# thuml/HashGAN

Measured on AMD Instinct MI355X. Metric: queries/sec (mAP@R of Q queries vs N-code database, Hamming ranking), higher is better.
Workload: dtype fp4 (E2M1 0/+-1) x fp4 -> f32 exact distances; u32 xor+popcount elsewhere; f64 AP; 1 GPU; C2: Q=10000 N=1000000 b=64 R=5000 C=10, planted codes; parallelism=1 GPU

## Files before the change

hashgan_amd/csrc/hg_core.hip:

```cpp
#include "hg_ctx.hpp"
#include "hg_host_pack.hpp"
#include "hg_dev_in.hpp"
#include "hg_dev_out.hpp"

#include <exception>
#include <map>
#include <mutex>
#include <thread>
#include <unistd.h>

thread_local std::string g_err;

int fail(int code, const char* fmt, ...) {
    char buf[512];
    va_list ap;
    va_start(ap, fmt);
    vsnprintf(buf, sizeof buf, fmt, ap);
    va_end(ap);
    g_err = buf;
    return code;
}

const char* const kKernelNames[KI_COUNT] = {"k_hist", "k_hist_reduce", "k_plan", "k_seg_counts", "k_seg_layout", "k_guess",
                                            "k_select", "k_rank_hist", "k_order", "k_rank_fused", "k_match", "k_ap", "k_merge", "k_pack",
// ... 1098 lines not shown
    flag("staged_lists", &Options::staged_lists),
    flag("step_graph", &Options::step_graph),
    ranged("step_streams", &Options::step_streams, 1, 2, "step_streams must be 1 or 2"),
    ranged("timing_every", &Options::timing_every, 1, 1024, "timing_every must be 1..1024"),
    flag("host_pack", &Options::host_pack),
    ranged("keep_floats", &Options::keep_floats, 0, 2, "keep_floats must be 0, 1 or 2"),
    ranged("keep_query_floats", &Options::keep_query_floats, 0, 1, "keep_query_floats must be 0 or 1"),
    ranged("real_mfma", &Options::real_mfma, 0, 2, "real_mfma must be 0, 1 or 2"),
    flag("real_sample_half", &Options::real_sample_half),
    flag("real_second_sample", &Options::real_second_sample),
    flag("real_sort_lds", &Options::real_sort_lds),
    flag("real_groups", &Options::real_groups),
    flag("real_map_lists", &Options::real_map_lists),
    ranged("real_whole_rounds", &Options::real_whole_rounds, 0, 8, "real_whole_rounds must be 0 .. 8"),
};
}

int hg_set_option(hg_ctx* c, const char* key, int64_t value) {
    if (!c || !key) return fail(HG_ERR_ARG, "hg_set_option: null argument");
    if (!strcmp(key, "handicap_next_bet")) {
        if (value < 0 || value > 64) return fail(HG_ERR_ARG, "handicap_next_bet must be 0..64");
        c->handicap_next = value;
        return HG_OK;
    }
    if (!strcmp(key, "optimistic")) {
        c->opt.optimistic = value != 0;
        c->bet_consecutive_fail = c->shard_bet_fail = 0;
        c->cfg_epoch++;
        return HG_OK;
    }
    if (!strcmp(key, "cap_boost")) {
        if (value < 1 || value > 4096) return fail(HG_ERR_ARG, "cap_boost must be 1..4096");
        if (value > c->cap_boost && c->shard_bet_fail > 0) c->shard_bet_fail--;
        c->cap_boost = value;
        c->cfg_epoch++;
        return HG_OK;
    }
    for (const OptionKey& k : kOptionKeys) {
        if (strcmp(key, k.key)) continue;
        if (!k.flag && (value < k.lo || value > k.hi)) return fail(HG_ERR_ARG, "%s", k.range);
        c->opt.*k.field = k.flag ? value != 0 : value;
        c->cfg_epoch++;
        return HG_OK;
    }
    return fail(HG_ERR_ARG, "hg_set_option: unknown key '%s'", key);
}

int hg_trim(hg_ctx* c) {
    if (!c) return fail(HG_ERR_ARG, "hg_trim: null context");
    HG_TRY(c->use());
    HG_TRY(c->sync());
    c->for_each_buf([](DevBuf& d, BufClass k) { if (k != BUF_TABLE) d.release(); });
    c->forget_derived();
    if (c->sub) { hg_ctx* s = c->sub; c->sub = nullptr; (void)hg_destroy(s); }
    c->stage &= (ST_DB | ST_Q);
    c->lists_valid = false;
    c->real_lists = false;
    cache_release_all();
    return HG_OK;
}

int hg_preload(hg_ctx* c) {
    if (!c) return fail(HG_ERR_ARG, "hg_preload: null context");
    HG_TRY(c->use());
    HG_TRY(ensure_stream2(c));
    HG_TRY(ensure_fstage(c));
    HG_TRY(ensure_pin(c, (size_t)1 << 20));
    hipFuncAttributes a;
    HG_HIP(hipFuncGetAttributes(&a, reinterpret_cast<const void*>(&k_ap<AP_THREADS>)));
    HG_TRY(preload_seq()); HG_TRY(preload_rank()); HG_TRY(preload_side()); HG_TRY(preload_valu()); HG_TRY(preload_mx()); HG_TRY(preload_mx1()); HG_TRY(preload_real()); HG_TRY(preload_rerank());
    host_pack_warm();
    return HG_OK;
}

int hg_release_cache(void) {
    cache_release_all();
    return HG_OK;
}

int hg_get_stat(hg_ctx* c, const char* key, int64_t* value) {
    if (!c || !key || !value) return fail(HG_ERR_ARG, "hg_get_stat: null argument");
    if (!strcmp(key, "optimistic_runs")) *value = c->bet_runs;
    else if (!strcmp(key, "optimistic_fallbacks")) *value = c->bet_fallbacks;
    else if (!strcmp(key, "optimistic_requeried")) *value = c->bet_requeried;
    else if (!strcmp(key, "optimistic_rebets")) *value = c->bet_rebets;
    else if (!strcmp(key, "rank_leftovers")) *value = c->rank_leftovers;
    else if (!strcmp(key, "select_variant")) *value = c->last_select;
    else if (!strcmp(key, "rank_variant")) *value = c->last_rank;
    else if (!strcmp(key, "hist_variant")) *value = c->last_hist;
    else if (!strcmp(key, "rank_lds_recs")) *value = c->last_lds_recs;
    else if (!strcmp(key, "slice_cap")) *value = c->cap;
    else if (!strcmp(key, "rel_hist_variant")) *value = c->last_rel_hist;
    else if (!strcmp(key, "ap_at_cutoffs")) *value = c->aa.dim;
    else if (!strcmp(key, "votes_cutoffs")) *value = c->vt.dim;
    else if (!strcmp(key, "joint_hist_grades")) *value = c->jh_G;
    else if (!strcmp(key, "joint_hist_bands")) *value = c->jh_bands;
    else if (!strcmp(key, "merged_joint_grades")) *value = c->mjh_G;
    else if (!strcmp(key, "rel_hist_current")) *value = c->rh.current(c) ? 1 : 0;
    else if (!strcmp(key, "grade_hist_current")) *value = c->gh.current(c) ? 1 : 0;
    else if (!strcmp(key, "joint_hist_current")) *value = c->jh.current(c) ? 1 : 0;
    else if (!strcmp(key, "rerank_records")) *value = c->rr_records;
    else if (!strcmp(key, "rerank_chunks")) *value = c->rr_chunks;
    else if (!strcmp(key, "rerank_groups_lds")) *value = c->rr_groups_lds;
    else if (!strcmp(key, "rerank_groups_global")) *value = c->rr_groups_global;
    else if (!strcmp(key, "export_bytes")) *value = c->export_bytes;
    else if (!strcmp(key, "export_variant")) *value = c->export_variant;
// ... 105 lines not shown
```

hashgan_amd/csrc/hg_ctx.hpp:

```cpp
#pragma once
#include "hg_kernels.hpp"
#pragma GCC visibility push(default)
#include "../../include/hashgan_amd.h"
#pragma GCC visibility pop

#include <rccl/rccl.h>
#include <atomic>
#include <chrono>
#include <cmath>
#include <cstdarg>
#include <cstdio>
#include <cstdlib>
#include <cstring>
#include <string>
#include <utility>
#include <vector>

using namespace hg;

extern thread_local std::string g_err;
int fail(int code, const char* fmt, ...);

#define HG_HIP(expr)                                                                         \
    do {                                                                                     \
// ... 167 lines not shown
    i64 min_segment = 256;
    i64 max_segments = 2048;
    i64 optimistic = 1;
    i64 sample_stride = 0;
    i64 guess_sigma = 5;
    i64 cand_budget_x10 = 40;
    i64 second_bet = 1;
    i64 crowd_probe = 1;
    i64 select_mfma = 1;
    i64 select_packed = 3;
    i64 compact_records = 1;
    i64 hist_mfma = 2;
    i64 rank_lds = 2;
    i64 rank_slices = 7000;
    i64 rank_dense = 1;
    i64 rank_dense_gbm = -1;
    i64 dense_budget_mb = 16384;
    i64 all_rows_shortcut = 1;
    i64 fuse_ap = 1;
    i64 inline_leftovers = 1;
    i64 ap_wide = 1;
    i64 ap_recip = 1;
    i64 probe_select = 0;
    i64 probe_votes = 0;
    i64 stage_sync = 1;
    i64 defer_verdict = 0;
    i64 staged_lists = 1;
    i64 step_graph = 0;
    i64 step_streams = 2;
    i64 timing_every = 1;
    i64 host_pack = 1;
    i64 keep_floats = 2;
    i64 keep_query_floats = 0;
    i64 real_mfma = 2;
    i64 real_sample_half = 1;
    i64 real_second_sample = 1;
    i64 real_sort_lds = 1;
    i64 real_groups = 1;
    i64 real_map_lists = 0;
    i64 real_whole_rounds = 3;
};

enum BufClass {
    BUF_TABLE,
    BUF_DERIVED,
    BUF_WORK,
};

struct StepBufs {
    DevBuf hist, hown, posbase, t, tguess, sstar, cnt_lt, quota, tie_before, n_lt, err, sl_start, sl_tie, sl_cnt, tot, failq,
           cand, out_idx, out_dist, mbits, ap, rel, qbad, bigq, hwq;
    DevBuf outblk;
    i64 outblk_q = -1;
    template <class F> void for_each_step_buf(F&& f) {
        for (DevBuf* d : {&hist, &hown, &posbase, &t, &tguess, &sstar, &cnt_lt, &quota, &tie_before, &n_lt, &err, &sl_start, &sl_tie,
                          &sl_cnt, &tot, &failq, &cand, &out_idx, &out_dist, &mbits, &ap, &rel, &qbad, &bigq, &hwq})
            f(*d, BUF_WORK);
        f(outblk, BUF_DERIVED);
    }
};

struct StepState {
    unsigned stage = ST_NONE;
    Geo geo{};
    i64 RW = 0;
    bool optimistic = false;
    bool lists_valid = false;
    bool rec8 = false;
    u32 cap = 0;
    i64 crow = 0;
    bool ap_fused = false;
    bool leftovers_inline = false;
    int last_select = SEL_NONE;
    int last_rank = RK_NONE;
    int last_hist = 0;
    i64 last_lds_recs = 0;
};

struct StepReq {
    bool fuse_ap = false;
    enum Rows { RECORDS, BYTES, DIRECT } rows = RECORDS;
    bool exact_cut = false;
    bool err_zeroed = false;
    i64 guess_sigma = 0;
    i64 cand_budget_x10 = 0;
    void* dst = nullptr;
};

struct RowSource;
struct RealReq {
    RowSource* src = nullptr;
    i64 R = 0;
    bool bet = false;
    double sigma = 0.0, budget = 0.0;
    bool with_ap = false;
    bool no_cut = false;
    double expect = 0.0;
    bool samp16 = false;
    bool skip_lists = false;
};

struct RealState {
    bool filtered = false;
    bool lds_ranked = false;
    bool grouped = false;
    bool lists_made = false;
    bool half = false;
    i64 attempts = 0;
// ... 295 lines not shown
inline void SideResult::finish(const hg_ctx* c, i64 Q_, i64 Qpad_, i64 dim_) { *this = SideResult{true, c->q_gen, c->db_gen, Q_, Qpad_, dim_}; }
inline bool SideResult::current(const hg_ctx* c) const { return done && q_gen == c->q_gen && db_gen == c->db_gen; }

struct FirstReservations {
    const unsigned long long e0 = g_alloc_epoch.load();
    void keep(hg_ctx* c) const { if (c->map_warm_epoch == e0) c->map_warm_epoch = g_alloc_epoch; }
};

inline int download_planes(hg_ctx* c, const DevBuf& src, size_t plane, void* const* host, int k) {
    for (int i = 0; i < k; ++i)
        if (host[i]) HG_HIP(hipMemcpyAsync(host[i], src.as<char>() + i * plane, plane, hipMemcpyDeviceToHost, c->stream));
    return HG_OK;
}
inline int download_pitched(hg_ctx* c, void* host, const DevBuf& src, i64 Q, i64 Qpad, i64 rows) {
    HG_HIP(hipMemcpy2DAsync(host, (size_t)Q * 4, src.p, (size_t)Qpad * 4, (size_t)Q * 4, (size_t)rows, hipMemcpyDeviceToHost, c->stream));
    return HG_OK;
}
inline void widen_u32(int64_t* dst, const void* src, size_t n) {
    for (size_t i = 0; i < n; ++i) dst[i] = ((const u32*)src)[i];
}

inline int grid_for(i64 n, int per_block = 256) { return (int)((n + per_block - 1) / per_block); }
inline int padded_grid(int nBlk) { return (nBlk + 7) / 8 * 8; }

int need(hg_ctx* c, unsigned st, const char* who, const char* what);
int upload_codes(hg_ctx* c, DevBuf& dst, const uint64_t* host, i64 n, int W, int NW);
int ensure_pin(hg_ctx* c, size_t need_b);
int do_match(hg_ctx* c);
int ensure_ap_tables(hg_ctx* c, bool* use_recip);
int do_ap_range(hg_ctx* c, i64 q0, i64 nq, const u32* only = nullptr);
inline int do_ap(hg_ctx* c) { return do_ap_range(c, 0, c->geo.Q); }
int ensure_out_block(hg_ctx* c);
int read_plan_flag(hg_ctx* c, int* flag);
int launch_min_topr(hg_ctx* c, const u32* idx_all, const u8* dist_all, i64 n, int G);
hg_ctx* requery_child(hg_ctx* c, i64 nF);
int stage_ap_download(hg_ctx* c, void* dst = nullptr);
int wait_verdict(hg_ctx* c, bool staged, int* flag);
Geo full_geometry(const hg_ctx* c);
inline void make_geometry(hg_ctx* c) { c->geo = full_geometry(c); }
Geo hist_geometry(const hg_ctx* c);
int set_R(hg_ctx* c, int64_t R, int G, int rank);
int rerank_hist_plan(hg_ctx* c, int64_t R);
int launch_rank(hg_ctx* c, RankMode mode, const StepReq& req);
int launch_rank_leftovers(hg_ctx* c);
int launch_order(hg_ctx* c);
bool rank_dense_fits(const hg_ctx* c);
inline bool lists_needed(const hg_ctx* c) { return c->want_lists || c->LW > 2; }
inline const int* cut_of(const hg_ctx* c, const StepReq& req) { return req.exact_cut ? c->t.as<int>() : c->tguess.as<int>(); }
int launch_hist(hg_ctx* c);
int launch_hist_rel(hg_ctx* c, const Geo& g);
int launch_select_valu(hg_ctx* c, int lw, bool optimistic);
int launch_select_dense(hg_ctx* c, int lw);
int ensure_mx_images(hg_ctx* c, bool need_db);
int launch_hist_mx(hg_ctx* c);
int launch_select_mx(hg_ctx* c, int lw, const int* cut);
int launch_select_mx3(hg_ctx* c, int lw, const int* cut);
int launch_select_mx4(hg_ctx* c, int lw, const int* cut);
int preload_valu(); int preload_mx(); int preload_mx1(); int preload_real(); int preload_seq(); int preload_rank(); int preload_side(); int preload_rerank();
void comm_release(hg_ctx* c);

#define HG_DISPATCH_NW(fn, c, ...)                              \
    switch ((c)->NW) {                                          \
        case 1: return fn<1>(c, ##__VA_ARGS__);                 \
        case 2: return fn<2>(c, ##__VA_ARGS__);                 \
        case 3: return fn<3>(c, ##__VA_ARGS__);                 \
        case 4: return fn<4>(c, ##__VA_ARGS__);                 \
        case 5: return fn<5>(c, ##__VA_ARGS__);                 \
        case 6: return fn<6>(c, ##__VA_ARGS__);                 \
        case 7: return fn<7>(c, ##__VA_ARGS__);                 \
        case 8: return fn<8>(c, ##__VA_ARGS__);                 \
        default: return fail(HG_ERR_ARG, "unsupported code length: %d words", (c)->NW); \
    }
```

hashgan_amd/csrc/hg_hist_i8.hpp:

```cpp
#pragma once
#include "hg_kernels.hpp"
#include "hg_hist_mx.hpp"

namespace hg {

typedef int i32x16 __attribute__((ext_vector_type(16)));
typedef __attribute__((address_space(3))) u32 lds_u32;

__device__ __forceinline__ void lds_add_at(const u32 addr, const u32 inc) {
#if defined(__HIP_DEVICE_COMPILE__)
    __hip_atomic_fetch_add((lds_u32*)addr, inc, __ATOMIC_RELAXED, __HIP_MEMORY_SCOPE_WORKGROUP);
#else
    (void)addr; (void)inc;
#endif
}

__device__ __forceinline__ uint4 bits16_to_bytes(const u32 bits, const u32 one, const u32 zero) {
    u32 w[4];
#pragma unroll
    for (int d = 0; d < 4; ++d) {
        u32 v = 0;
#pragma unroll
        for (int i = 0; i < 4; ++i) v |= (((bits >> (4 * d + i)) & 1u) ? one : zero) << (8 * i);
        w[d] = v;
    }
    return uint4{w[0], w[1], w[2], w[3]};
}

static __global__ __launch_bounds__(256) void k_expand_db_i8(const u32* __restrict__ db, uint4* __restrict__ img, i64 N, i64 n16, int NW) {
    const i64 i = (i64)blockIdx.x * 256 + threadIdx.x;
    if (i >= n16 * NW * 2) return;
    const i64 row = i / (NW * 2);
    const int c = (int)(i - row * NW * 2), m = c >> 1, hh = c & 1;
    const u32 word = row < N ? db[row * NW + m] : 0u;
    img[(((row >> 4) * NW + m) * 2 + hh) * 16 + (row & 15)] = bits16_to_bytes((word >> (16 * hh)) & 0xFFFFu, 8u, 0u);
}

constexpr int hist_i8_cols(bool pack16) { return pack16 ? 1 : 2; }

template <int NW, bool PACK16>
__global__ __launch_bounds__(256) __attribute__((amdgpu_waves_per_eu(4, 4)))
void k_hist_i8(const u32* __restrict__ qc, const u8* __restrict__ dbx8, u32* __restrict__ hist, const Geo g) {
    extern __shared__ __attribute__((aligned(16))) u32 hlds[];
    constexpr int QT = 2, WQ = 32 * QT;
    const int lb = logical_block(g.nBlk);
    if (lb < 0) return;
    const int lane = threadIdx.x & 63;
    const int wave = __builtin_amdgcn_readfirstlane(threadIdx.x >> 6);
    const int nQB = g.nQT;
    const int sp = lb / nQB, qb = lb - sp * nQB;
    const int h = lane >> 5, j = lane & 31;
    const int NB = g.NB, b = g.NB - 1;
    const i64 lo0 = (i64)(2 * sp) * g.L, lo1 = lo0 + g.L;
    const i64 len0 = (lo0 + g.L < g.N ? g.L : g.N - lo0);
    const i64 len1 = lo1 >= g.N ? 0 : (lo1 + g.L < g.N ? g.L : g.N - lo1);
    const i64 mylen = h ? len1 : len0;
    const i64 ntile = ((len0 > len1 ? len0 : len1) + 15) / 16;
    const i64 NG = (g.N + 15) >> 4;
    const int stride = g.hist_stride;

    constexpr int NCOL = hist_i8_cols(PACK16);
    u32* col = hlds + wave * NCOL * NB * 32;
    for (int i = lane; i < NCOL * NB * 32; i += 64) col[i] = 0u;

    const int q0w = (qb * WPB + wave) * WQ;
    i32x4 bq[QT][NW];
    i32x16 biasv[QT];
    u32 inc[QT];
#pragma unroll
    for (int t = 0; t < QT; ++t) {
        const int q = q0w + t * 32 + j;
        int pop = 0;
#pragma unroll
        for (int m = 0; m < NW; ++m) {
            const u32 word = q < g.Q ? qc[(i64)q * NW + m] : 0u;
            pop += __builtin_popcount(word);
            const int first = 32 * m + 16 * h;
            const u32 valid = b - first >= 16 ? 0xFFFFu : (b - first <= 0 ? 0u : (1u << (b - first)) - 1u);
            const u32 bits = (word >> (16 * h)) & 0xFFFFu;
            const uint4 neg = bits16_to_bytes(bits & valid, 0xF0u, 0u);
            const uint4 pos = bits16_to_bytes(~bits & valid, 0x10u, 0u);
            bq[t][m] = i32x4{(int)(neg.x | pos.x), (int)(neg.y | pos.y), (int)(neg.z | pos.z), (int)(neg.w | pos.w)};
        }
        u32* c0 = col + (PACK16 ? 0 : t * NB * 32) + j;
        const int base = (int)(u32)(size_t)(lds_u32*)c0 + 128 * pop;
#pragma unroll
        for (int r = 0; r < 16; ++r) biasv[t][r] = base;
        inc[t] = PACK16 ? (t ? 65536u : 1u) : 1u;
    }
    wave_lds_sync();

    const int ah = (j >> 2) & 1;
    const int ar = (j & 3) + 4 * (j >> 3);
    const i64 ag0 = (ah ? lo1 : lo0) >> 4;
    auto chunk = [&](const i64 T, const int m) -> i32x4 {
        i64 G = ag0 + T;
        G = G < NG ? G : NG - 1;
        return *(const i32x4*)(dbx8 + ((((G * NW + m) * 2 + h) * 16 + ar) * 16));
    };
    i32x4 av[NW];
    if (ntile > 0) {
#pragma unroll
        for (int m = 0; m < NW; ++m) av[m] = chunk(0, m);
    }
    for (i64 T = 0; T < ntile; T += stride) {
        i32x4 an[NW];
        const i64 Tn = T + stride < ntile ? T + stride : T;
#pragma unroll
        for (int m = 0; m < NW; ++m) an[m] = chunk(Tn, m);
        const i64 left = mylen - T * 16;
        const bool whole = __all(left >= 16);
#pragma unroll
        for (int t = 0; t < QT; ++t) {
            i32x16 acc = biasv[t];
#pragma unroll
            for (int m = 0; m < NW; ++m) acc = __builtin_amdgcn_mfma_i32_32x32x32_i8(av[m], bq[t][m], acc, 0, 0, 0);
            if (whole) {
#pragma unroll
                for (int r = 0; r < 16; ++r)
                    lds_add_at((u32)acc[r], inc[t]);
            } else {
#pragma unroll
                for (int r = 0; r < 16; ++r)
                    if ((i64)r < left) lds_add_at((u32)acc[r], inc[t]);
            }
        }
#pragma unroll
        for (int m = 0; m < NW; ++m) av[m] = an[m];
    }
    wave_lds_sync();
    const int q = q0w + lane;
    if (q < g.Qpad) {
        u32* __restrict__ out = hist + (i64)sp * NB * g.Qpad + q;
        const int dn = g.hcap > 0 && g.hcap < NB ? g.hcap : NB;
        for (int d = 0; d < dn; ++d) {
            const u32 v = PACK16 ? (col[d * 32 + j] >> (16 * h)) & 0xFFFFu : col[(h * NB + d) * 32 + j];
            out[(i64)d * g.Qpad] = v;
        }
    }
}

}
```

hashgan_amd/csrc/hg_kernels.hpp:

```cpp
#pragma once
#include <hip/hip_runtime.h>
#include <stdint.h>

namespace hg {

typedef uint32_t u32;
typedef uint64_t u64;
typedef unsigned char u8;
typedef long long i64;

constexpr int WPB = 4;
constexpr u32 IDX_NONE = 0xFFFFFFFFu;
constexpr int AP_CHUNK = 8192;
constexpr int AP_LEAF = 128;
constexpr int AP_THREADS = 128;
constexpr int TAIL_WORDS = 64;
#ifndef HG_PROBES
#define HG_PROBES 0
#endif
constexpr bool kProbes = HG_PROBES != 0;

struct Geo {
    int Q, Qpad, nQT;
    int NW, NB;
// ... 201 lines not shown
        if (keep) last = s;
        pos += lt + keep;
        tierank += tie;
    }
    tot[q] = pos;
    if (sstar && q < g.Q) sstar[q] = last < 0 ? -1 : (last + 1) * ratio - 1;
}

static __global__ __launch_bounds__(256) void k_guess(const u32* __restrict__ hs, const u32* __restrict__ hall, int G, int rank,
                                               const u32* __restrict__ hseg, int Sh, int ratio,
                                               double sigma, i64 n_total, int* __restrict__ T, int* __restrict__ sstar,
                                               const Geo g) {
    const int q = blockIdx.x * 256 + threadIdx.x;
    if (q >= g.Q) return;
    const i64 plane = (i64)g.NB * g.Qpad + TAIL_WORDS;
    u64 sampled = 0;
    if (G > 1) for (int r = 0; r < G; ++r) sampled += hall[(i64)r * plane + plane - TAIL_WORDS + 1];
    else sampled = hs[plane - TAIL_WORDS + 1];
    const double fr = (double)g.R * (double)sampled / (double)n_total;
    const double needd = fr + sigma * sqrt(fr) + 1.0;
    const u64 need = (u64)ceil(needd);
    u64 cum = 0, below = 0;
    int t = g.NB - 1;
    bool found = false;
    for (int d = 0; d < g.NB; ++d) {
        const i64 o = (i64)d * g.Qpad + q;
        below = cum;
        if (G > 1) for (int r = 0; r < G; ++r) cum += hall[(i64)r * plane + o];
        else cum += hs[o];
        if (cum >= need) { t = d; found = true; break; }
    }
    T[q] = t;
    int ss = g.S - 1;
    if (found) {
        u64 have = below;
        const i64 ot = (i64)t * g.Qpad + q;
        if (G > 1) for (int r = 0; r < rank; ++r) have += hall[(i64)r * plane + ot];
        if (have >= need) {
            ss = -1;
        } else {
            for (int sh = 0; sh < Sh; ++sh) {
                have += hseg[((i64)sh * g.NB + t) * g.Qpad + q];
                if (have >= need) { ss = (sh + 1) * ratio - 1; break; }
            }
            if (ss > g.S - 1) ss = g.S - 1;
        }
    }
    sstar[q] = ss;
}

template <int PARTS>
__global__ __launch_bounds__(256) void k_guess_direct(const u32* __restrict__ hseg, int Sh, int ratio, double sigma,
                                                      i64 n_total, u32 sampled, int* __restrict__ T, int* __restrict__ sstar,
                                                      u32* __restrict__ failq, int* __restrict__ err, u32* __restrict__ crowd, const Geo g) {
    constexpr int QPW = 64 / PARTS;
    const int lane = threadIdx.x & 63, part = lane / QPW;
    const int q = (blockIdx.x * WPB + (threadIdx.x >> 6)) * QPW + (lane % QPW);
    if (part == 0 && q < g.Qpad) failq[q] = 0u;
    if (q == 0 && part == 0) { err[0] = 0; err[1] = 0; }
    const bool live = q < g.Q;
    const int qq = live ? q : 0;
    const double fr = (double)g.R * (double)sampled / (double)n_total;
    const u64 need = (u64)ceil(fmax(1.0, fr + sigma * sqrt(fr) + 1.0));
    const i64 plane = (i64)g.NB * g.Qpad;
    const int per = (Sh + PARTS - 1) / PARTS;
    const int s0 = part * per < Sh ? part * per : Sh, s1 = s0 + per < Sh ? s0 + per : Sh;
    u64 cum = 0, below = 0;
    int t = g.NB - 1;
    bool found = false;
    const int dn = g.hcap > 0 && g.hcap < g.NB ? g.hcap : g.NB;
    constexpr int PL = 4;
    u32 gmax = 0, gtot = 0;
    for (int d = 0; d < dn && !found; d += PL) {
        u32 cs[PL];
        const u32* __restrict__ col[PL];
        gmax = 0;
#pragma unroll
        for (int p = 0; p < PL; ++p) { cs[p] = 0; col[p] = hseg + (i64)(d + p < dn ? d + p : d) * g.Qpad + qq; }
        for (int sh = s0; sh < s1; sh += 8) {
            u32 v[PL][8];
#pragma unroll
            for (int k = 0; k < 8; ++k) {
                const i64 o = (i64)(sh + k < s1 ? sh + k : 0) * plane;
#pragma unroll
                for (int p = 0; p < PL; ++p) v[p][k] = col[p][o];
            }
#pragma unroll
            for (int k = 0; k < 8; ++k) {
                u32 sk = 0;
#pragma unroll
                for (int p = 0; p < PL; ++p) { const u32 x = sh + k < s1 ? v[p][k] : 0u; cs[p] += x; sk += x; }
                gmax = sk > gmax ? sk : gmax;
            }
        }
#pragma unroll
        for (int off = QPW; off < 64; off <<= 1)
#pragma unroll
            for (int p = 0; p < PL; ++p) cs[p] += (u32)__shfl_xor((int)cs[p], off);
        gtot = 0;
#pragma unroll
        for (int p = 0; p < PL; ++p) {
            gtot += cs[p];
            if (!found && d + p < dn) {
                below = cum;
                cum += cs[p];
                if (cum >= need) { t = d + p; found = true; }
            }
        }
    }
    if (crowd) {
#pragma unroll
        for (int off = QPW; off < 64; off <<= 1) {
            const u32 m = (u32)__shfl_xor((int)gmax, off);
            gmax = gmax > m ? gmax : m;
        }
        if (live && found && part == 0) { atomicAdd(crowd, gmax); atomicAdd(crowd + 1, gtot); }
    }
    int ss = g.S - 1;
    if (found) {
        const u32* __restrict__ col = hseg + (i64)t * g.Qpad + qq;
        u32 mine = 0;
        for (int sh = s0; sh < s1; ++sh) mine += col[(i64)sh * plane];
        u32 incl = mine;
#pragma unroll
        for (int off = QPW; off < 64; off <<= 1) {
            const u32 v = (u32)__shfl_up((int)incl, off);
            if (lane >= off) incl += v;
        }
        u64 have = below + (u64)(incl - mine);
        int cand = 0x7FFFFFFF;
        for (int sh = s0; sh < s1; ++sh) {
            have += col[(i64)sh * plane];
            if (have >= need) { cand = sh; break; }
        }
#pragma unroll
        for (int off = QPW; off < 64; off <<= 1) {
            const int m = __shfl_xor(cand, off);
            cand = cand < m ? cand : m;
        }
        if (cand != 0x7FFFFFFF) ss = (cand + 1) * ratio - 1;
        if (ss > g.S - 1) ss = g.S - 1;
    }
    if (live && part == 0) { T[q] = t; sstar[q] = ss; }
}

struct SelArgs {
    const int* T;
    const u32* sl_start;
    const u32* sl_tie;
    u32* sl_cnt;
    u32* fail;
    u32 cap;
    i64 crow;
    int optimistic;
    const int* sstar;
    int probe;
};

constexpr int sel_batch_rows(int nw) {
    int r = 64 / nw, p = 1;
    while (p * 2 <= r) p *= 2;
    return p > 32 ? 32 : (p < 2 ? 2 : p);
}

__device__ __forceinline__ u64 make_rec(u32 idx, u32 d, bool m) {
    return (u64)idx | ((u64)(d | (m ? 0x100u : 0u)) << 32);
}

template <int NW, int LW, bool OPT>
__global__ __launch_bounds__(256) void k_select(const u32* __restrict__ qc, const u64* __restrict__ qlab,
                                                const u32* __restrict__ db, const u64* __restrict__ dblab,
                                                const SelArgs a, u64* __restrict__ cand, const Geo g) {
    const int lb = logical_block(g.nBlk);
    if (lb < 0) return;
    const int lane = threadIdx.x & 63;
    const int wave = __builtin_amdgcn_readfirstlane(threadIdx.x >> 6);
    const i64 unit = (i64)lb * g.wpb + wave;
    if (unit >= g.nUnits) return;
    const int s = (int)(unit / g.nQT);
    const int qt = (int)(unit - (i64)s * g.nQT);
    const int q = qt * 64 + lane;
    const bool live = q < g.Q;
    constexpr int LWA = LW > 0 ? LW : 1;

    u32 qw[NW];
#pragma unroll
    for (int w = 0; w < NW; ++w) qw[w] = live ? qc[(i64)q * NW + w] : 0u;
    u64 ql[LWA];
#pragma unroll
    for (int w = 0; w < LWA; ++w) ql[w] = (LW > 0 && live) ? qlab[(i64)q * LW + w] : 0ull;
    const int T = live ? (OPT ? a.T[q] - (s > a.sstar[q] ? 1 : 0) : a.T[q]) : -1;
    const u32 bias = (u32)(-T - 1);
    const i64 so = (i64)s * g.Qpad + q;
    u32 start, tielim = 0xFFFFFFFFu;
    if (OPT) start = (u32)s * a.cap;
    else { start = a.sl_start[so]; tielim = a.sl_tie[so]; }
// ... 1100 lines not shown
```

hashgan_amd/csrc/hg_pairs_mx.hip:

```cpp
#include "hg_ctx.hpp"
#include "hg_mx_drain.hpp"
#include "hg_select_mx.hpp"
#include "hg_select_mx3.hpp"
#include "hg_select_mx4.hpp"
#include "hg_hist_mx.hpp"
#include "hg_hist_i8.hpp"

int ensure_mx_images(hg_ctx* c, const bool need_db) {
    const int NW = c->NW, NM = (NW + 1) / 2;
    if (need_db && !c->dbx_valid) {
        const i64 n16 = (c->N + 15) / 16 * 16;
        HG_TRY(c->dbx.reserve((size_t)(n16 > 0 ? n16 : 16) * NM * 32));
        const i64 items = n16 * 2 * NM;
        c->t_begin(KI_PACK);
        if (items) hipLaunchKernelGGL(k_expand_db, dim3(grid_for(items)), dim3(256), 0, c->stream, c->db.as<u32>(),
                                      c->dbx.as<uint4>(), (i64)c->N, n16, NW, NM);
        c->t_end();
        HG_TRY(c->check_launch("k_expand_db"));
        c->dbx_valid = true;
    }
    if (!c->qx_valid) {
        const i64 qpad = ((i64)c->Q + 511) / 512 * 512;
        HG_TRY(c->qx.reserve((size_t)qpad * NM * 32));
        const i64 items = qpad * 2 * NM;
// ... 27 lines not shown
    if (pack16) {
        hipLaunchKernelGGL((k_hist_mx<NW, true>), dim3(padded_grid(g.nBlk)), dim3(256), lds, c->stream, c->qc.as<u32>(), c->qx.as<u8>(),
                           c->dbx.as<u8>(), c->hist.as<u32>(), g);
    } else {
        if (lds > 64 * 1024)
            HG_HIP(hipFuncSetAttribute(reinterpret_cast<const void*>(&k_hist_mx<NW, false>), hipFuncAttributeMaxDynamicSharedMemorySize, (int)lds));
        hipLaunchKernelGGL((k_hist_mx<NW, false>), dim3(padded_grid(g.nBlk)), dim3(256), lds, c->stream, c->qc.as<u32>(), c->qx.as<u8>(),
                           c->dbx.as<u8>(), c->hist.as<u32>(), g);
    }
    c->t_end();
    return c->check_launch("k_hist_mx");
}

template <class P, class Expand, class Kernel>
int launch_select_packed(hg_ctx* c, const int* cut, const int NW, const int LW, DevBuf& image, bool& image_valid, Expand expand,
                         const char* expand_name, Kernel kernel, const char* kernel_name) {
    HG_TRY(ensure_mx_images(c, false));
    if (!image_valid) {
        const i64 n = (c->N + P::ROWS - 1) / P::ROWS * P::ROWS + P::WS_MAX * P::ROWS;
        HG_TRY(image.reserve((size_t)n * P::IMG_WORDS * 16));
        const i64 items = n * P::IMG_WORDS;
        c->t_begin(KI_PACK);
        hipLaunchKernelGGL(expand, dim3(grid_for(items)), dim3(256), 0, c->stream, c->db.as<u32>(), image.as<uint4>(), (i64)c->N, n, NW);
        c->t_end();
        HG_TRY(c->check_launch(expand_name));
        image_valid = true;
    }
    Geo g = c->geo;
    const int nSP = (g.S + 1) / 2;
    const int nQB = (g.Q + 64 * P::WPB - 1) / (64 * P::WPB);
    g.nQT = nQB;
    g.nUnits = (i64)nSP * nQB;
    g.wpb = P::WPB;
    g.nBlk = (int)g.nUnits;
    const PackedLds L = packed_lds_layout<P>(NW, LW);
    if (L.total > 64 * 1024)
        HG_HIP(hipFuncSetAttribute(reinterpret_cast<const void*>(kernel), hipFuncAttributeMaxDynamicSharedMemorySize, L.total));
    SelArgs a{cut, c->sl_start.as<u32>(), c->sl_tie.as<u32>(), c->sl_cnt.as<u32>(),
              c->failq.as<u32>(), c->cap, c->crow, 1, c->sstar.as<int>(), (int)c->opt.probe_select};
    c->t_begin(KI_SELECT_MX);
    hipLaunchKernelGGL(kernel, dim3(padded_grid(g.nBlk)), dim3(64 * P::WPB), (size_t)L.total, c->stream, c->qc.as<u32>(),
                       c->qlab.as<u64>(), c->qx.as<u8>(), c->db.as<u32>(), image.as<u8>(), c->dblab.as<u64>(), a,
                       c->cand.as<u8>(), g);
    c->t_end();
    return c->check_launch(kernel_name);
}
template <int NW, int LW> int launch_select_mx3_t(hg_ctx* c, const int* cut) {
    return launch_select_packed<M3Pack>(c, cut, NW, LW, c->dbx3, c->dbx3_valid, k_expand_db3, "k_expand_db3", &k_select_mx3<NW, LW>, "k_select_mx3");
}
template <int NW, int LW> int launch_select_mx4_t(hg_ctx* c, const int* cut) {
    return launch_select_packed<M4Pack>(c, cut, NW, LW, c->dbx4, c->dbx4_valid, k_expand_db4, "k_expand_db4", &k_select_mx4<NW, LW>, "k_select_mx4");
}

template <int NW> int launch_hist_i8_t(hg_ctx* c) {
    if (!c->dbx8_valid) {
        const i64 n16 = (c->N + 15) / 16 * 16;
        HG_TRY(c->dbx8.reserve((size_t)n16 * NW * 32));
        c->t_begin(KI_PACK);
        hipLaunchKernelGGL(k_expand_db_i8, dim3(grid_for(n16 * NW * 2)), dim3(256), 0, c->stream, c->db.as<u32>(), c->dbx8.as<uint4>(),
                           (i64)c->N, n16, NW);
        c->t_end();
        HG_TRY(c->check_launch("k_expand_db_i8"));
        c->dbx8_valid = true;
    }
    Geo g = c->geo;
    const int nSP = (g.S + 1) / 2;
    const int nQB = (g.Q + 255) / 256;
    g.nQT = nQB;
    g.nUnits = (i64)nSP * nQB;
    g.wpb = WPB;
    g.nBlk = (int)g.nUnits;
    const i64 tiles_per_half = ((g.L + 15) / 16 + g.hist_stride - 1) / g.hist_stride;
    const bool pack16 = 2 * tiles_per_half * 16 < 65536;
    const size_t lds = (size_t)WPB * hist_i8_cols(pack16) * g.NB * 32 * 4;
    c->last_hist = pack16 ? 3 : 7;
    c->t_begin(KI_HIST);
    if (pack16) {
        if (lds > 64 * 1024)
            HG_HIP(hipFuncSetAttribute(reinterpret_cast<const void*>(&k_hist_i8<NW, true>), hipFuncAttributeMaxDynamicSharedMemorySize, (int)lds));
        hipLaunchKernelGGL((k_hist_i8<NW, true>), dim3(padded_grid(g.nBlk)), dim3(256), lds, c->stream, c->qc.as<u32>(), c->dbx8.as<u8>(),
                           c->hist.as<u32>(), g);
    } else {
        if (lds > 64 * 1024)
            HG_HIP(hipFuncSetAttribute(reinterpret_cast<const void*>(&k_hist_i8<NW, false>), hipFuncAttributeMaxDynamicSharedMemorySize, (int)lds));
        hipLaunchKernelGGL((k_hist_i8<NW, false>), dim3(padded_grid(g.nBlk)), dim3(256), lds, c->stream, c->qc.as<u32>(), c->dbx8.as<u8>(),
                           c->hist.as<u32>(), g);
    }
    c->t_end();
    return c->check_launch("k_hist_i8");
}
}

int launch_hist_mx(hg_ctx* c) {
    if (c->opt.hist_mfma == 2 && c->NW <= 4) {
        switch (c->NW) {
            case 1: return launch_hist_i8_t<1>(c);
            case 2: return launch_hist_i8_t<2>(c);
            case 3: return launch_hist_i8_t<3>(c);
            default: return launch_hist_i8_t<4>(c);
        }
    }
    HG_DISPATCH_NW(launch_hist_mx_t, c)
}


int launch_select_mx4(hg_ctx* c, int lw, const int* cut) {
    if (c->NW < 3 || c->NW > 4 || lw < 1 || lw > 2) return fail(HG_ERR_ARG, "k_select_mx4 takes codes of 65..128 bits and 1..128 classes");
    if (c->NW == 3) return lw == 1 ? launch_select_mx4_t<3, 1>(c, cut) : launch_select_mx4_t<3, 2>(c, cut);
    return lw == 1 ? launch_select_mx4_t<4, 1>(c, cut) : launch_select_mx4_t<4, 2>(c, cut);
}

int launch_select_mx3(hg_ctx* c, int lw, const int* cut) {
    if (c->NW > 2 || lw < 1 || lw > 2) return fail(HG_ERR_ARG, "k_select_mx3 takes codes of <= 64 bits and 1..128 classes");
    if (c->NW == 1) return lw == 1 ? launch_select_mx3_t<1, 1>(c, cut) : launch_select_mx3_t<1, 2>(c, cut);
    return lw == 1 ? launch_select_mx3_t<2, 1>(c, cut) : launch_select_mx3_t<2, 2>(c, cut);
}

int preload_mx() {
    hipFuncAttributes a;
    HG_HIP(hipFuncGetAttributes(&a, reinterpret_cast<const void*>(&k_select_mx3<2, 1>)));
    return HG_OK;
}
```

hashgan_amd/csrc/hg_seq.hip:

```cpp
#include "hg_ctx.hpp"
#include "hg_select_mx.hpp"
#include "hg_select_mx3.hpp"
#include "hg_select_mx4.hpp"
#include "hg_hist_mx.hpp"

constexpr i64 SAMPLE_RATIO = 2;

Geo full_geometry(const hg_ctx* c) {
    Geo g = c->geo;
    g.Q = (int)c->Q;
    g.nQT = (int)((c->Q + 63) / 64);
    g.Qpad = g.nQT * 64;
    g.NW = c->NW; g.NB = c->NB; g.LW = c->LW;
    g.N = c->N; g.R = c->R; g.idx_base = c->idx_base;
    i64 S = (c->opt.target_units + g.nQT - 1) / g.nQT;
    if (S > c->opt.max_segments) S = c->opt.max_segments;
    const i64 maxS = (c->N + c->opt.min_segment - 1) / c->opt.min_segment;
    if (S > maxS) S = maxS;
    if (S < 1) S = 1;
    i64 L = (c->N + S - 1) / S;
    const i64 lq = (c->opt.select_packed >= 3 && c->NW <= 2) ? 96 : 32;
    L = (L + lq - 1) / lq * lq;
    if (L < lq) L = lq;
    S = (c->N + L - 1) / L;
// ... 59 lines not shown
    return select_takes_mx(c) && c->opt.compact_records && !c->want_lists && c->LW <= 2 && c->cap % 16 == 0 && c->crow * 64 < (1ll << 31);
}
static int reserve_records(hg_ctx* c) {
    return c->cand.reserve((size_t)c->geo.Q * (size_t)c->crow * (records_are_bytes(c) ? 1 : 8) + 64);
}

static int launch_select(hg_ctx* c, const StepReq& req) {
    const int NW = c->NW;
    const int* cut = cut_of(c, req);
    const int lw = c->LW <= 2 ? c->LW : 0;
    const bool mx = select_takes_mx(c);
    c->rec8 = records_are_bytes(c);
    if (!c->optimistic && c->R * 4 >= c->n_total) { c->last_select = SEL_DENSE; return launch_select_dense(c, lw); }
    if (NW <= 2 && c->opt.select_packed == 3 && c->rec8 && c->geo.L % M3_ROWS == 0 && (lw == 1 || lw == 2)) { c->last_select = SEL_MX3; return launch_select_mx3(c, lw, cut); }
    if ((NW == 3 || NW == 4) && c->opt.select_packed == 3 && c->rec8 && c->geo.L % M4_ROWS == 0 && (lw == 1 || lw == 2)) { c->last_select = SEL_MX4; return launch_select_mx4(c, lw, cut); }
    if (mx) { c->last_select = SEL_MX; return launch_select_mx(c, lw, cut); }
    c->last_select = SEL_VALU;
    return launch_select_valu(c, lw, c->optimistic);
}

template <int NW> i64 sampled_rows_t(Geo g, int stride, int ratio) {
    g.hist_stride = stride;
    {
        const i64 L = g.L * ratio;
        g.L = L;
        g.S = (int)((g.N + L - 1) / L);
    }
    constexpr int B = Batch<NW>::rows;
    i64 total = 0;
    for (int s = 0; s < g.S; ++s) {
        const i64 lo = (i64)s * g.L, hi = lo + g.L < g.N ? lo + g.L : g.N;
        const i64 nb = (hi - lo) / B;
        total += (nb + stride - 1) / stride * B;
    }
    return total;
}
i64 sampled_rows(hg_ctx* c, int stride) {
    if (hist_mx_applies(c, stride, false)) return hist_mx_sampled_rows(c->geo, stride);
    switch (c->NW) {
        case 1: return sampled_rows_t<1>(c->geo, stride, (int)SAMPLE_RATIO);
        case 2: return sampled_rows_t<2>(c->geo, stride, (int)SAMPLE_RATIO);
        case 3: return sampled_rows_t<3>(c->geo, stride, (int)SAMPLE_RATIO);
        case 4: return sampled_rows_t<4>(c->geo, stride, (int)SAMPLE_RATIO);
        case 5: return sampled_rows_t<5>(c->geo, stride, (int)SAMPLE_RATIO);
        case 6: return sampled_rows_t<6>(c->geo, stride, (int)SAMPLE_RATIO);
        case 7: return sampled_rows_t<7>(c->geo, stride, (int)SAMPLE_RATIO);
        default: return sampled_rows_t<8>(c->geo, stride, (int)SAMPLE_RATIO);
    }
}


extern "C" {

static int do_hist(hg_ctx* c, int stride, bool reduce = true, bool pairs_ok = false, int hcap = 0) {
    make_geometry(c);
    c->geo.hist_stride = stride;
    const bool mx = hist_mx_applies(c, stride, pairs_ok);
    c->geo.hcap = mx && !reduce && stride > 1 ? hcap : 0;
    c->hist_pairs = mx && stride == 1;
    const Geo& g = c->geo;
    const size_t plane = (size_t)g.NB * g.Qpad * 4;
    HG_TRY(c->hist.reserve(plane * g.S));
    HG_TRY(c->hown.reserve(plane + TAIL_WORDS * 4));
    if (reduce) {
        const u32 visited = (u32)(stride == 1 ? g.N : sampled_rows(c, stride));
        hipLaunchKernelGGL(k_set_tail, dim3(1), dim3(64), 0, c->stream, (u32*)(c->hown.as<char>() + plane), visited);
        HG_TRY(c->check_launch("k_set_tail"));
    }
    HG_TRY(mx ? launch_hist_mx(c) : launch_hist(c));
    if (!reduce) { c->stage = ST_DB | ST_Q; return HG_OK; }
    const Geo gh = hist_geometry(c);
    c->t_begin(KI_HIST_REDUCE);
    hipLaunchKernelGGL(k_hist_reduce, dim3(grid_for((i64)g.NB * g.Qpad)), dim3(256), 0, c->stream,
                       c->hist.as<u32>(), c->hown.as<u32>(), gh);
    c->t_end();
    HG_TRY(c->check_launch("k_hist_reduce"));
    c->stage = ST_DB | ST_Q | (stride == 1 ? ST_HIST : 0);
    return HG_OK;
}

int hg_hist(hg_ctx* c) {
    HG_TRY(need(c, ST_DB | ST_Q, "hg_hist", "hg_set_database + hg_set_queries"));
    HG_TRY(do_hist(c, 1));
    return c->stage_end();
}

int hg_hist_buffer(hg_ctx* c, void** dev_ptr, int64_t* nbytes) {
    HG_TRY(need(c, ST_DB | ST_Q, "hg_hist_buffer", "hg_hist / hg_sample_hist / hg_select_candidates"));
    if (!c->hown.p) return fail(HG_ERR_STATE, "hg_hist_buffer: no histogram computed yet");
    if (dev_ptr) *dev_ptr = c->hown.p;
    if (nbytes) *nbytes = ((int64_t)c->geo.NB * c->geo.Qpad + TAIL_WORDS) * 4;
    return HG_OK;
}

extern "C++" int set_R(hg_ctx* c, int64_t R, int G, int rank) {
    if (G < 1 || rank < 0 || rank >= G) return fail(HG_ERR_ARG, "rank %d of %d", rank, G);
    if (R < 1 || R > c->n_total)
        return fail(HG_ERR_ARG, "R=%lld outside 1..N (N=%lld rows in the database)", (long long)R, (long long)c->n_total);
    c->R = R; c->G = G; c->rank = rank;
    c->lists_changed();
    c->bitmap_changed();
    c->mbits_merged = c->mbits_in_ws_b = false;
    c->rr.begin();
    c->geo.R = R;
    c->RW = (R + 63) / 64;
    return HG_OK;
}

static int launch_plan(hg_ctx* c, const uint32_t* dev_hist_all) {
    const Geo& g = c->geo;
    const size_t qb = (size_t)g.Qpad * 4;
    HG_TRY(c->posbase.reserve((size_t)g.NB * qb));
    HG_TRY(c->t.reserve(qb)); HG_TRY(c->cnt_lt.reserve(qb)); HG_TRY(c->quota.reserve(qb));
    HG_TRY(c->tie_before.reserve(qb)); HG_TRY(c->n_lt.reserve(qb)); HG_TRY(c->err.reserve(16));
    HG_HIP(hipMemsetAsync(c->err.p, 0, 4, c->stream));
    Plan pl{c->t.as<int>(), c->cnt_lt.as<u32>(), c->quota.as<u32>(), c->tie_before.as<u32>(), c->n_lt.as<u32>(),
            c->posbase.as<u32>(), c->err.as<int>()};
    c->t_begin(KI_PLAN);
    hipLaunchKernelGGL(k_plan, dim3(grid_for(g.Q)), dim3(256), 0, c->stream, c->hown.as<u32>(),
                       (const u32*)dev_hist_all, c->G, c->rank, pl, g);
    c->t_end();
    return c->check_launch("k_plan");
// ... 446 lines not shown
}

static int enqueue_all_rows(hg_ctx* c, int64_t R, const StepReq& req, StepReq::Rows rows) {
    make_geometry(c);
    HG_TRY(set_R(c, R, 1, 0));
    const Geo& g = c->geo;
    const size_t qb = (size_t)g.Qpad * 4;
    HG_TRY(c->err.reserve(16)); HG_TRY(c->failq.reserve(qb)); HG_TRY(c->tot.reserve(qb)); HG_TRY(c->sl_cnt.reserve(qb));
    HG_TRY(c->cand.reserve(64));
    HG_TRY(reserve_lists(c, c->want_lists, FILL_NONE));
    HG_HIP(hipMemsetAsync(c->err.p, 0, 4, c->stream));
    c->optimistic = false;
    c->crow = R;
    c->cap = 0;
    c->rec8 = false;
    c->last_select = SEL_NONE;
    StepReq walk = req;
    walk.rows = rows;
    HG_TRY(launch_rank(c, RANK_WHOLE, walk));
    c->lists_valid = c->want_lists;
    c->stage = ST_DB | ST_Q | ST_PLAN | ST_SELECT | ST_MATCH;
    return HG_OK;
}

static int enqueue_exact(hg_ctx* c, int64_t R, const StepReq& req) {
    if (R * 8 > c->N && c->opt.all_rows_shortcut && rank_dense_fits(c)) return enqueue_all_rows(c, R, req, StepReq::BYTES);
    if (c->N == c->n_total && R == c->N && c->opt.all_rows_shortcut && c->LW <= 2 && c->NW <= 8)
        return enqueue_all_rows(c, R, req, StepReq::DIRECT);
    HG_TRY(do_hist(c, 1));
    HG_TRY(do_plan(c, R, nullptr, 1, 0));
    return do_select(c, req);
}

static bool exact_mx_applies(const hg_ctx* c, int64_t R) {
    return c->opt.select_mfma && c->N == c->n_total && R * 8 <= c->N && c->N >= 65536 && !c->is_sub;
}
static int enqueue_exact_mx(hg_ctx* c, int64_t R, const StepReq& req) {
    HG_TRY(do_hist(c, 1, true, true));
    HG_TRY(do_plan(c, R, nullptr, 1, 0));
    const Geo& g = c->geo;
    const double mean = 0.1 * (double)c->opt.cand_budget_x10 * (double)R / (double)g.S;
    u32 cap = (u32)std::ceil(mean + 6.0 * std::sqrt(mean) + 16.0);
    cap = (cap + 15u) & ~15u;
    c->optimistic = true;
    c->cap = cap;
    c->crow = (i64)g.S * cap;
    HG_HIP(hipMemsetAsync(c->failq.p, 0, (size_t)g.Qpad * 4, c->stream));
    StepReq exact = req;
    exact.exact_cut = true;
    return do_select(c, exact);
}

static int enqueue_optimistic(hg_ctx* c, int64_t R, int stride, const StepReq& req) {
    HG_TRY(do_hist(c, stride, false, false, c->NB / 2 + 2));
    HG_TRY(set_R(c, R, 1, 0));
    const Geo& g = c->geo;
    HG_TRY(reserve_guess(c));
    HG_TRY(c->err.reserve(16));
    const bool probe = c->opt.crowd_probe && !c->crowd_probed && c->cap_boost == 1 && !c->capturing && !c->is_sub;
    u32* crowd = probe ? c->err.as<u32>() + 2 : nullptr;
    if (probe) HG_HIP(hipMemsetAsync(crowd, 0, 8, c->stream));
    c->t_begin(KI_GUESS);
    const Geo gh = hist_geometry(c);
    {
        const int ratio = (int)(gh.L / g.L);
        const u32 srows = (u32)sampled_rows(c, stride);
        double sigma = (double)req.guess_sigma;
        if (c->handicap_next && !c->capturing) { sigma = -(double)c->handicap_next; c->handicap_next = 0; }
#define HG_GUESS(P)                                                                                                     \
        hipLaunchKernelGGL(k_guess_direct<P>, dim3(grid_for(g.Qpad, WPB * (64 / P))), dim3(256), 0, c->stream,          \
                           c->hist.as<u32>(), gh.S, ratio, sigma, (i64)c->n_total, srows,                \
                           c->tguess.as<int>(), c->sstar.as<int>(), c->failq.as<u32>(), c->err.as<int>(), crowd, g)
        if (gh.S <= 64) HG_GUESS(4);
        else if (gh.S <= 512) HG_GUESS(16);
        else HG_GUESS(64);
#undef HG_GUESS
    }
    c->t_end();
    HG_TRY(c->check_launch("k_guess_direct"));
    if (probe) {
        u32 cr[2] = {0u, 0u};
        HG_HIP(hipMemcpyAsync(cr, crowd, 8, hipMemcpyDeviceToHost, c->stream));
        HG_TRY(c->sync());
        c->crowd_probed = true;
        const double ratio = cr[1] ? (double)cr[0] * (double)gh.S / (double)cr[1] : 0.0;
        c->crowd_x100 = (i64)(ratio * 100.0);
        if (ratio > 4.0) {
            i64 boost = 2;
            while ((double)boost < ratio && boost < 64) boost *= 2;
            c->cap_boost = boost;
            c->cfg_epoch++;
        }
    }
    adopt_guess(c, 0.1 * (double)req.cand_budget_x10 * (double)c->cap_boost * (double)R / (double)g.S);
    StepReq guessed = req;
    guessed.err_zeroed = true;
    return do_select(c, guessed);
}

static int rerun_lost_queries(hg_ctx* c, int64_t R, bool lists, bool with_ap, bool* handled) {
    *handled = false;
    const Geo g = c->geo;
    std::vector<u32> bad((size_t)g.Q);
    HG_HIP(hipMemcpyAsync(bad.data(), c->qbad.p, (size_t)g.Q * 4, hipMemcpyDeviceToHost, c->stream));
    HG_TRY(c->sync());
    std::vector<u32> lost;
    for (int q = 0; q < g.Q; ++q) if (bad[(size_t)q]) lost.push_back((u32)q);
    const i64 nF = (i64)lost.size();
    if (nF == 0 || nF * 8 > g.Q) return HG_OK;
    hg_ctx* s = requery_child(c, nF);
    s->opt.optimistic = 0;
    s->opt.max_segments = 256;
    HG_TRY(c->flist.reserve((size_t)nF * 4));
    HG_HIP(hipMemcpyAsync(c->flist.p, lost.data(), (size_t)nF * 4, hipMemcpyHostToDevice, c->stream));
    HG_TRY(s->qc.reserve((size_t)nF * c->NW * 4 + 64 * 4));
    HG_TRY(s->qlab.reserve((size_t)nF * c->LW * 8));
    auto move = [&](const void* src, void* dst, i64 rowbytes, int gather) {
        hipLaunchKernelGGL(k_move_rows, dim3((unsigned)nF), dim3(256), 0, c->stream, (const u8*)src, (u8*)dst,
                           c->flist.as<u32>(), rowbytes, gather);
    };
    move(c->qc.p, s->qc.p, (i64)c->NW * 4, 1);
    move(c->qlab.p, s->qlab.p, (i64)c->LW * 8, 1);
    HG_TRY(c->check_launch("k_move_rows"));
    s->stage = ST_DB | ST_Q;
    s->want_lists = lists;
    HG_TRY(enqueue_exact(s, R, StepReq{}));
    if (with_ap) HG_TRY(do_ap(s));
    move(s->mbits.p, c->mbits.p, c->RW * 8, 0);
    if (with_ap) {
        move(s->ap.p, c->ap.p, 8, 0);
        move(s->rel.p, c->rel.p, 4, 0);
    }
// ... 374 lines not shown
```

Baseline: 12.48 million queries/s.

## Accumulate per-distance histogram totals in hist kernel to shortcut guess walk

The int8 histogram kernel now atomically adds per-query, per-distance-pair totals, packed as two u32 values in a u64, into a new totals buffer while writing out its segmented histograms. k_guess_direct then scans these precomputed totals to find the threshold distance, instead of walking all segment planes for every distance. It also caches the per-segment values of the chosen distance in registers, and re-zeroes the totals buffer afterwards so the next call needs no memset. This trades global atomics in the hist kernel and an extra buffer for far fewer strided reads in the guess kernel.

```diff
diff --git a/hashgan_amd/csrc/hg_core.hip b/hashgan_amd/csrc/hg_core.hip
--- a/hashgan_amd/csrc/hg_core.hip
+++ b/hashgan_amd/csrc/hg_core.hip
@@ -1174,6 +1174,7 @@
     HG_TRY(c->sync());
     c->for_each_buf([](DevBuf& d, BufClass k) { if (k != BUF_TABLE) d.release(); });
     c->forget_derived();
+    c->hist_tot_zero = c->ws_b.hist_tot_zero = nullptr;
     if (c->sub) { hg_ctx* s = c->sub; c->sub = nullptr; (void)hg_destroy(s); }
     c->stage &= (ST_DB | ST_Q);
     c->lists_valid = false;
diff --git a/hashgan_amd/csrc/hg_ctx.hpp b/hashgan_amd/csrc/hg_ctx.hpp
--- a/hashgan_amd/csrc/hg_ctx.hpp
+++ b/hashgan_amd/csrc/hg_ctx.hpp
@@ -243,8 +243,10 @@
            cand, out_idx, out_dist, mbits, ap, rel, qbad, bigq, hwq;
     DevBuf outblk;
     i64 outblk_q = -1;
+    DevBuf hist_tot;
+    const void* hist_tot_zero = nullptr;
     template <class F> void for_each_step_buf(F&& f) {
-        for (DevBuf* d : {&hist, &hown, &posbase, &t, &tguess, &sstar, &cnt_lt, &quota, &tie_before, &n_lt, &err, &sl_start, &sl_tie,
+        for (DevBuf* d : {&hist_tot, &hist, &hown, &posbase, &t, &tguess, &sstar, &cnt_lt, &quota, &tie_before, &n_lt, &err, &sl_start, &sl_tie,
                           &sl_cnt, &tot, &failq, &cand, &out_idx, &out_dist, &mbits, &ap, &rel, &qbad, &bigq, &hwq})
             f(*d, BUF_WORK);
         f(outblk, BUF_DERIVED);
@@ -646,7 +648,8 @@
 int launch_select_valu(hg_ctx* c, int lw, bool optimistic);
 int launch_select_dense(hg_ctx* c, int lw);
 int ensure_mx_images(hg_ctx* c, bool need_db);
-int launch_hist_mx(hg_ctx* c);
+int launch_hist_mx(hg_ctx* c, u64* tot = nullptr);
+bool hist_i8_applies(const hg_ctx* c);
 int launch_select_mx(hg_ctx* c, int lw, const int* cut);
 int launch_select_mx3(hg_ctx* c, int lw, const int* cut);
 int launch_select_mx4(hg_ctx* c, int lw, const int* cut);
diff --git a/hashgan_amd/csrc/hg_hist_i8.hpp b/hashgan_amd/csrc/hg_hist_i8.hpp
--- a/hashgan_amd/csrc/hg_hist_i8.hpp
+++ b/hashgan_amd/csrc/hg_hist_i8.hpp
@@ -40,7 +40,7 @@
 
 template <int NW, bool PACK16>
 __global__ __launch_bounds__(256) __attribute__((amdgpu_waves_per_eu(4, 4)))
-void k_hist_i8(const u32* __restrict__ qc, const u8* __restrict__ dbx8, u32* __restrict__ hist, const Geo g) {
+void k_hist_i8(const u32* __restrict__ qc, const u8* __restrict__ dbx8, u32* __restrict__ hist, u64* __restrict__ tot, const Geo g) {
     extern __shared__ __attribute__((aligned(16))) u32 hlds[];
     constexpr int QT = 2, WQ = 32 * QT;
     const int lb = logical_block(g.nBlk);
@@ -133,9 +133,17 @@
     if (q < g.Qpad) {
         u32* __restrict__ out = hist + (i64)sp * NB * g.Qpad + q;
         const int dn = g.hcap > 0 && g.hcap < NB ? g.hcap : NB;
-        for (int d = 0; d < dn; ++d) {
-            const u32 v = PACK16 ? (col[d * 32 + j] >> (16 * h)) & 0xFFFFu : col[(h * NB + d) * 32 + j];
-            out[(i64)d * g.Qpad] = v;
+        for (int d = 0; d < dn; d += 2) {
+            u32 v[2] = {0u, 0u};
+#pragma unroll
+            for (int e = 0; e < 2; ++e) {
+                if (d + e < dn) {
+                    v[e] = PACK16 ? (col[(d + e) * 32 + j] >> (16 * h)) & 0xFFFFu : col[(h * NB + d + e) * 32 + j];
+                    out[(i64)(d + e) * g.Qpad] = v[e];
+                }
+            }
+            if (tot && (v[0] | v[1]) && q < g.Q)
+                __hip_atomic_fetch_add(tot + (i64)(d >> 1) * g.Qpad + q, (u64)v[0] | ((u64)v[1] << 32), __ATOMIC_RELAXED, __HIP_MEMORY_SCOPE_AGENT);
         }
     }
 }
diff --git a/hashgan_amd/csrc/hg_kernels.hpp b/hashgan_amd/csrc/hg_kernels.hpp
--- a/hashgan_amd/csrc/hg_kernels.hpp
+++ b/hashgan_amd/csrc/hg_kernels.hpp
@@ -277,7 +277,7 @@
 template <int PARTS>
 __global__ __launch_bounds__(256) void k_guess_direct(const u32* __restrict__ hseg, int Sh, int ratio, double sigma,
                                                       i64 n_total, u32 sampled, int* __restrict__ T, int* __restrict__ sstar,
-                                                      u32* __restrict__ failq, int* __restrict__ err, u32* __restrict__ crowd, const Geo g) {
+                                                      u32* __restrict__ failq, int* __restrict__ err, u32* __restrict__ crowd, u64* tot, const Geo g) {
     constexpr int QPW = 64 / PARTS;
     const int lane = threadIdx.x & 63, part = lane / QPW;
     const int q = (blockIdx.x * WPB + (threadIdx.x >> 6)) * QPW + (lane % QPW);
@@ -296,7 +296,24 @@
     const int dn = g.hcap > 0 && g.hcap < g.NB ? g.hcap : g.NB;
     constexpr int PL = 4;
     u32 gmax = 0, gtot = 0;
-    for (int d = 0; d < dn && !found; d += PL) {
+    const bool walk = !tot || crowd;
+    const int dn2 = (dn + 1) >> 1;
+    constexpr int TL = 18;
+    for (int d2 = 0; !walk && d2 < dn2 && !found; d2 += TL) {
+        u64 v[TL];
+#pragma unroll
+        for (int p = 0; p < TL; ++p) v[p] = tot[(i64)(d2 + p < dn2 ? d2 + p : dn2 - 1) * g.Qpad + qq];
+#pragma unroll
+        for (int p = 0; p < 2 * TL; ++p) {
+            const int d = 2 * d2 + p;
+            if (live && !found && d < dn) {
+                below = cum;
+                cum += (u32)(v[p >> 1] >> (32 * (p & 1)));
+                if (cum >= need) { t = d; found = true; }
+            }
+        }
+    }
+    for (int d = 0; walk && d < dn && !found; d += PL) {
         u32 cs[PL];
         const u32* __restrict__ col[PL];
         gmax = 0;
@@ -344,8 +361,18 @@
     int ss = g.S - 1;
     if (found) {
         const u32* __restrict__ col = hseg + (i64)t * g.Qpad + qq;
+        constexpr int SR = 16;
+        const bool inreg = per <= SR;
+        u32 cv[SR];
+#pragma unroll
+        for (int k = 0; k < SR; ++k) cv[k] = inreg ? col[(i64)(s0 + k < s1 ? s0 + k : 0) * plane] : 0u;
         u32 mine = 0;
-        for (int sh = s0; sh < s1; ++sh) mine += col[(i64)sh * plane];
+        if (inreg) {
+#pragma unroll
+            for (int k = 0; k < SR; ++k) mine += s0 + k < s1 ? cv[k] : 0u;
+        } else {
+            for (int sh = s0; sh < s1; ++sh) mine += col[(i64)sh * plane];
+        }
         u32 incl = mine;
 #pragma unroll
         for (int off = QPW; off < 64; off <<= 1) {
@@ -354,9 +381,19 @@
         }
         u64 have = below + (u64)(incl - mine);
         int cand = 0x7FFFFFFF;
-        for (int sh = s0; sh < s1; ++sh) {
-            have += col[(i64)sh * plane];
-            if (have >= need) { cand = sh; break; }
+        if (inreg) {
+#pragma unroll
+            for (int k = 0; k < SR; ++k) {
+                if (cand == 0x7FFFFFFF && s0 + k < s1) {
+                    have += cv[k];
+                    if (have >= need) cand = s0 + k;
+                }
+            }
+        } else {
+            for (int sh = s0; sh < s1; ++sh) {
+                have += col[(i64)sh * plane];
+                if (have >= need) { cand = sh; break; }
+            }
         }
 #pragma unroll
         for (int off = QPW; off < 64; off <<= 1) {
@@ -367,6 +404,8 @@
         if (ss > g.S - 1) ss = g.S - 1;
     }
     if (live && part == 0) { T[q] = t; sstar[q] = ss; }
+    if (tot && q < g.Qpad)
+        for (int d2 = part; d2 < dn2; d2 += PARTS) tot[(i64)d2 * g.Qpad + q] = 0ull;
 }
 
 struct SelArgs {
diff --git a/hashgan_amd/csrc/hg_pairs_mx.hip b/hashgan_amd/csrc/hg_pairs_mx.hip
--- a/hashgan_amd/csrc/hg_pairs_mx.hip
+++ b/hashgan_amd/csrc/hg_pairs_mx.hip
@@ -103,7 +103,7 @@
     return launch_select_packed<M4Pack>(c, cut, NW, LW, c->dbx4, c->dbx4_valid, k_expand_db4, "k_expand_db4", &k_select_mx4<NW, LW>, "k_select_mx4");
 }
 
-template <int NW> int launch_hist_i8_t(hg_ctx* c) {
+template <int NW> int launch_hist_i8_t(hg_ctx* c, u64* tot) {
     if (!c->dbx8_valid) {
         const i64 n16 = (c->N + 15) / 16 * 16;
         HG_TRY(c->dbx8.reserve((size_t)n16 * NW * 32));
@@ -130,27 +130,30 @@
         if (lds > 64 * 1024)
             HG_HIP(hipFuncSetAttribute(reinterpret_cast<const void*>(&k_hist_i8<NW, true>), hipFuncAttributeMaxDynamicSharedMemorySize, (int)lds));
         hipLaunchKernelGGL((k_hist_i8<NW, true>), dim3(padded_grid(g.nBlk)), dim3(256), lds, c->stream, c->qc.as<u32>(), c->dbx8.as<u8>(),
-                           c->hist.as<u32>(), g);
+                           c->hist.as<u32>(), tot, g);
     } else {
         if (lds > 64 * 1024)
             HG_HIP(hipFuncSetAttribute(reinterpret_cast<const void*>(&k_hist_i8<NW, false>), hipFuncAttributeMaxDynamicSharedMemorySize, (int)lds));
         hipLaunchKernelGGL((k_hist_i8<NW, false>), dim3(padded_grid(g.nBlk)), dim3(256), lds, c->stream, c->qc.as<u32>(), c->dbx8.as<u8>(),
-                           c->hist.as<u32>(), g);
+                           c->hist.as<u32>(), tot, g);
     }
     c->t_end();
     return c->check_launch("k_hist_i8");
 }
 }
 
-int launch_hist_mx(hg_ctx* c) {
-    if (c->opt.hist_mfma == 2 && c->NW <= 4) {
+bool hist_i8_applies(const hg_ctx* c) { return c->opt.hist_mfma == 2 && c->NW <= 4; }
+
+int launch_hist_mx(hg_ctx* c, u64* tot) {
+    if (hist_i8_applies(c)) {
         switch (c->NW) {
-            case 1: return launch_hist_i8_t<1>(c);
-            case 2: return launch_hist_i8_t<2>(c);
-            case 3: return launch_hist_i8_t<3>(c);
-            default: return launch_hist_i8_t<4>(c);
+            case 1: return launch_hist_i8_t<1>(c, tot);
+            case 2: return launch_hist_i8_t<2>(c, tot);
+            case 3: return launch_hist_i8_t<3>(c, tot);
+            default: return launch_hist_i8_t<4>(c, tot);
         }
     }
+    if (tot) return fail(HG_ERR_STATE, "launch_hist_mx: plane totals come from k_hist_i8 only");
     HG_DISPATCH_NW(launch_hist_mx_t, c)
 }
 
diff --git a/hashgan_amd/csrc/hg_seq.hip b/hashgan_amd/csrc/hg_seq.hip
--- a/hashgan_amd/csrc/hg_seq.hip
+++ b/hashgan_amd/csrc/hg_seq.hip
@@ -135,7 +135,11 @@
 
 extern "C" {
 
-static int do_hist(hg_ctx* c, int stride, bool reduce = true, bool pairs_ok = false, int hcap = 0) {
+#ifndef HG_GUESS_TOTALS
+#define HG_GUESS_TOTALS 1
+#endif
+
+static int do_hist(hg_ctx* c, int stride, bool reduce = true, bool pairs_ok = false, int hcap = 0, u64** tot_out = nullptr) {
     make_geometry(c);
     c->geo.hist_stride = stride;
     const bool mx = hist_mx_applies(c, stride, pairs_ok);
@@ -144,13 +148,24 @@
     const Geo& g = c->geo;
     const size_t plane = (size_t)g.NB * g.Qpad * 4;
     HG_TRY(c->hist.reserve(plane * g.S));
+    u64* tot = nullptr;
+    if (tot_out) *tot_out = nullptr;
+    if (HG_GUESS_TOTALS && tot_out && mx && hist_i8_applies(c) && c->N == c->n_total && !c->is_sub) {
+        const int dn = g.hcap > 0 && g.hcap < g.NB ? g.hcap : g.NB;
+        const size_t cap0 = c->hist_tot.cap;
+        HG_TRY(c->hist_tot.reserve((size_t)((dn + 1) / 2) * g.Qpad * 8));
+        if (c->hist_tot_zero != c->hist_tot.p || c->hist_tot.cap != cap0)
+            HG_HIP(hipMemsetAsync(c->hist_tot.p, 0, c->hist_tot.cap, c->stream));
+        c->hist_tot_zero = nullptr;
+        *tot_out = tot = c->hist_tot.as<u64>();
+    }
     HG_TRY(c->hown.reserve(plane + TAIL_WORDS * 4));
     if (reduce) {
         const u32 visited = (u32)(stride == 1 ? g.N : sampled_rows(c, stride));
         hipLaunchKernelGGL(k_set_tail, dim3(1), dim3(64), 0, c->stream, (u32*)(c->hown.as<char>() + plane), visited);
         HG_TRY(c->check_launch("k_set_tail"));
     }
-    HG_TRY(mx ? launch_hist_mx(c) : launch_hist(c));
+    HG_TRY(mx ? launch_hist_mx(c, tot) : launch_hist(c));
     if (!reduce) { c->stage = ST_DB | ST_Q; return HG_OK; }
     const Geo gh = hist_geometry(c);
     c->t_begin(KI_HIST_REDUCE);
@@ -703,7 +718,8 @@
 }
 
 static int enqueue_optimistic(hg_ctx* c, int64_t R, int stride, const StepReq& req) {
-    HG_TRY(do_hist(c, stride, false, false, c->NB / 2 + 2));
+    u64* tot = nullptr;
+    HG_TRY(do_hist(c, stride, false, false, c->NB / 2 + 2, &tot));
     HG_TRY(set_R(c, R, 1, 0));
     const Geo& g = c->geo;
     HG_TRY(reserve_guess(c));
@@ -721,7 +737,7 @@
 #define HG_GUESS(P)                                                                                                     \
         hipLaunchKernelGGL(k_guess_direct<P>, dim3(grid_for(g.Qpad, WPB * (64 / P))), dim3(256), 0, c->stream,          \
                            c->hist.as<u32>(), gh.S, ratio, sigma, (i64)c->n_total, srows,                \
-                           c->tguess.as<int>(), c->sstar.as<int>(), c->failq.as<u32>(), c->err.as<int>(), crowd, g)
+                           c->tguess.as<int>(), c->sstar.as<int>(), c->failq.as<u32>(), c->err.as<int>(), crowd, tot, g)
         if (gh.S <= 64) HG_GUESS(4);
         else if (gh.S <= 512) HG_GUESS(16);
         else HG_GUESS(64);
@@ -729,6 +745,7 @@
     }
     c->t_end();
     HG_TRY(c->check_launch("k_guess_direct"));
+    if (tot) c->hist_tot_zero = tot;
     if (probe) {
         u32 cr[2] = {0u, 0u};
         HG_HIP(hipMemcpyAsync(cr, crowd, 8, hipMemcpyDeviceToHost, c->stream));
```

Measured after the change: 12.65 million queries/s, median of 6. 1.4% higher.
